# nfmoore/databricks-kubernetes-mlops-poc

Hardware: AMD Instinct MI355X
Metric: requests/sec (whole node), credit-default /score, bs=1024 (higher is better)
Workload: dtype fp32; 1 GPU; model=RandomForest 500xdepth16 + IForest100 + TabularDrift, global_batch=1024, request_rows=1024, with_drift=True, train_rows=20000, parallelism=dp1, device=cuda

## Files before the change

csrc/creditcore_kernels.hip:

```cpp

#include <torch/extension.h>

#include <c10/hip/HIPGuard.h>
#include <c10/hip/HIPStream.h>
#include <hip/hip_runtime.h>

#define BLOCK 256
#define N_CAT 9
#define N_NUM 14
#define MAX_DRIFT_ROWS 16384
static constexpr size_t KS_LDS_BYTES_MAX = 160 * 1024 - 1024;

#define HIP_CHECK(expr)                                              \
  do {                                                               \
    hipError_t _e = (expr);                                          \
    TORCH_CHECK(_e == hipSuccess, "HIP error: ", hipGetErrorString(_e)); \
  } while (0)


template <bool DIRECT>
__global__ __launch_bounds__(BLOCK) void forest_kernel(
    const short* __restrict__ codes,
    const float* __restrict__ nums,
    const float* __restrict__ medians,
// ... 88 lines not shown
    const int ta = t;
    const int tb = t + gridDim.y;
    const int basea = tree_off[ta];
    int4 na = nodes[basea];
    bool la = true;
    int baseb = 0;
    int4 nb;
    bool lb = tb < n_trees;
    if (lb) { baseb = tree_off[tb]; nb = nodes[baseb]; }
    while (la || lb) {
      if (la) {
        if (na.x >= 0) {
          const float v = value_of(na.x);
          na = nodes[basea + ((v <= __int_as_float(na.y)) ? na.z : na.w)];
        } else {
          local += (double)__int_as_float(na.y);
          la = false;
        }
      }
      if (lb) {
        if (nb.x >= 0) {
          const float v = value_of(nb.x);
          nb = nodes[baseb + ((v <= __int_as_float(nb.y)) ? nb.z : nb.w)];
        } else {
          local += (double)__int_as_float(nb.y);
          lb = false;
        }
      }
    }
  }
  atomicAdd(&acc[row], local);
}

template <bool DIRECT>
__device__ __forceinline__ double forest_walk_ilp2(
    const short* __restrict__ s_codes,
    const float* __restrict__ s_nums,
    int tid,
    const int4* __restrict__ nodes,
    const int* __restrict__ tree_off,
    int n_trees,
    const int* __restrict__ feat_col,
    const int* __restrict__ feat_code,
    int chunk,
    int n_chunks)
{
  auto value_of = [&](int f) -> float {
    if (DIRECT) return s_nums[f * BLOCK + tid];
    const int col = feat_col[f];
    const int code = feat_code[f];
    return (code >= 0) ? ((s_codes[col * BLOCK + tid] == (short)code) ? 1.0f : 0.0f)
                       : s_nums[col * BLOCK + tid];
  };
  double local = 0.0;
  for (int t = chunk; t < n_trees; t += 2 * n_chunks) {
    const int ta = t;
    const int tb = t + n_chunks;
    const int basea = tree_off[ta];
    int4 na = nodes[basea];
    bool la = true;
    int baseb = 0;
    int4 nb;
    bool lb = tb < n_trees;
    if (lb) { baseb = tree_off[tb]; nb = nodes[baseb]; }
    while (la || lb) {
      if (la) {
        if (na.x >= 0) {
          const float v = value_of(na.x);
          na = nodes[basea + ((v <= __int_as_float(na.y)) ? na.z : na.w)];
        } else {
          local += (double)__int_as_float(na.y);
          la = false;
        }
      }
      if (lb) {
        if (nb.x >= 0) {
          const float v = value_of(nb.x);
          nb = nodes[baseb + ((v <= __int_as_float(nb.y)) ? nb.z : nb.w)];
        } else {
          local += (double)__int_as_float(nb.y);
          lb = false;
        }
      }
    }
  }
  return local;
}

__global__ __launch_bounds__(BLOCK) void forest_kernel_dual(
    const short* __restrict__ codes,
    const float* __restrict__ nums,
    const float* __restrict__ medians,
    const int4* __restrict__ cls_nodes,
    const int* __restrict__ cls_off,
    int t_cls,
    const int* __restrict__ feat_col,
    const int* __restrict__ feat_code,
    const int4* __restrict__ if_nodes,
    const int* __restrict__ if_off,
    int t_if,
    int chunks_cls,
    int n_rows,
    double* __restrict__ acc_cls,
    double* __restrict__ acc_if)
{
  __shared__ short s_codes[N_CAT * BLOCK];
  __shared__ float s_nums[N_NUM * BLOCK];
  const int tid = threadIdx.x;
  const int row = blockIdx.x * BLOCK + tid;
  const bool is_cls = (int)blockIdx.y < chunks_cls;
  if (row < n_rows) {
    if (is_cls) {
#pragma unroll
      for (int c = 0; c < N_CAT; ++c) s_codes[c * BLOCK + tid] = codes[row * N_CAT + c];
    }
#pragma unroll
    for (int c = 0; c < N_NUM; ++c) {
      const float v = nums[row * N_NUM + c];
      s_nums[c * BLOCK + tid] = isnan(v) ? medians[c] : v;
    }
  }
  if (row >= n_rows) return;
  if (is_cls) {
    const double local = forest_walk_ilp2<false>(
        s_codes, s_nums, tid, cls_nodes, cls_off, t_cls, feat_col, feat_code,
        blockIdx.y, chunks_cls);
    atomicAdd(&acc_cls[row], local);
  } else {
    const double local = forest_walk_ilp2<true>(
        s_codes, s_nums, tid, if_nodes, if_off, t_if, nullptr, nullptr,
        blockIdx.y - chunks_cls, gridDim.y - chunks_cls);
    atomicAdd(&acc_if[row], local);
  }
}

#define CONTRIB_BLOCK 128
#define N_SRC (N_CAT + N_NUM)

__global__ __launch_bounds__(CONTRIB_BLOCK) void forest_contrib_kernel(
    const short* __restrict__ codes,
    const float* __restrict__ nums,
    const float* __restrict__ medians,
    const int4* __restrict__ nodes,
    const float* __restrict__ node_value,
    const int* __restrict__ tree_off,
    int n_trees,
    const int* __restrict__ feat_col,
    const int* __restrict__ feat_code,
    int n_rows,
    double scale,
    double* __restrict__ contrib)
{
  __shared__ double s_acc[N_SRC * CONTRIB_BLOCK];
  __shared__ short s_codes[N_CAT * CONTRIB_BLOCK];
  __shared__ float s_nums[N_NUM * CONTRIB_BLOCK];

  const int tid = threadIdx.x;
  const int row = blockIdx.x * CONTRIB_BLOCK + tid;
  if (row >= n_rows) return;

#pragma unroll
  for (int c = 0; c < N_CAT; ++c)
// ... 2225 lines not shown
  TORCH_CHECK(B <= MAX_DRIFT_ROWS, "K-S batch too large: ", B);
  TORCH_CHECK((int)rs_off.size(0) == F + 1, "rs_off size mismatch");
  TORCH_CHECK(block == 256 || block == 512, "block must be 256 or 512");
  auto ks_d = torch::empty({F},
      torch::TensorOptions().dtype(torch::kFloat32).device(nums.device()));
  hipStream_t stream = c10::hip::getCurrentHIPStream();
  int m_pow2 = (int)block / 64;
  while (m_pow2 < B) m_pow2 <<= 1;
  size_t smem = (size_t)m_pow2 * sizeof(float);
  auto rs_off64 = rs_off.to(torch::kInt64);
  if (ref_lds) {
    int64_t maxr = 0;
    auto ro = rs_off64.cpu();
    auto* rp = ro.data_ptr<int64_t>();
    for (int j = 0; j < F; ++j) maxr = std::max<int64_t>(maxr, rp[j + 1] - rp[j]);
    smem += (size_t)maxr * sizeof(float);
    TORCH_CHECK(smem <= KS_LDS_BYTES_MAX, "ref too large for LDS");
  }
  if (block == 512)
    hipLaunchKernelGGL((ks_kernel_t<512>), dim3(F), dim3(512), smem, stream,
        nums.data_ptr<float>(), medians.data_ptr<float>(), F, B, m_pow2,
        (int)ref_lds, ref_sorted.data_ptr<float>(),
        rs_off64.data_ptr<int64_t>(), ks_d.data_ptr<float>());
  else
    hipLaunchKernelGGL((ks_kernel_t<256>), dim3(F), dim3(256), smem, stream,
        nums.data_ptr<float>(), medians.data_ptr<float>(), F, B, m_pow2,
        (int)ref_lds, ref_sorted.data_ptr<float>(),
        rs_off64.data_ptr<int64_t>(), ks_d.data_ptr<float>());
  HIP_CHECK(hipGetLastError());
  return ks_d;
}


inline bool spin_sync_enabled() {
  static const bool on = (std::getenv("CREDITCORE_BLOCK_SYNC") == nullptr);
  return on;
}

inline void sync_stream(hipStream_t s) {
  if (spin_sync_enabled()) {
    hipError_t e;
    while ((e = hipStreamQuery(s)) == hipErrorNotReady) {}
    if (e != hipSuccess) HIP_CHECK(e);
  } else {
    HIP_CHECK(hipStreamSynchronize(s));
  }
}

inline void sync_event(hipEvent_t ev) {
  static const bool spin = (std::getenv("CREDITCORE_SPIN_EVENT") != nullptr);
  if (spin) {
    hipError_t e;
    while ((e = hipEventQuery(ev)) == hipErrorNotReady) {}
    if (e != hipSuccess) HIP_CHECK(e);
  } else {
    HIP_CHECK(hipEventSynchronize(ev));
  }
}

struct ScoreSession {
  torch::Tensor cls_nodes, cls_off, feat_col, feat_code, medians;
  torch::Tensor if_nodes, if_off, ref_sorted, rs_off, cat_off;
  torch::Tensor d_codes, d_nums, acc, outs, d_drift, d_ks_scratch;
  size_t drift_bytes = 0, drift_ksd_off = 0;
  torch::Tensor pin_codes, pin_nums, pin_outs, pin_drift;
  torch::Tensor pin_hist, pin_ksd;
  double if_denom{}, if_offset{}, if_threshold{};
  int cls_kind{};
  double cls_bias{};
  int64_t total_bins{}, t_cls{}, t_if{}, capacity{};
  int device_index{};
  hipStream_t stream{};
  hipStream_t stream2{};
  hipEvent_t ev_fork{}, ev_join{};
  hipEvent_t ev_done[2]{};

  int16_t* p_codes(int s) { return pin_codes.data_ptr<int16_t>() + (size_t)s * capacity * N_CAT; }
  float* p_nums(int s) { return pin_nums.data_ptr<float>() + (size_t)s * capacity * N_NUM; }
  double* p_outs(int s) { return pin_outs.data_ptr<double>() + (size_t)s * 3 * capacity; }
  uint8_t* p_drift(int s) { return pin_drift.data_ptr<uint8_t>() + (size_t)s * drift_bytes; }
  int32_t* p_hist(int s) { return reinterpret_cast<int32_t*>(p_drift(s)); }
  float* p_ksd(int s) { return reinterpret_cast<float*>(p_drift(s) + drift_ksd_off); }
  int32_t* d_hist() { return reinterpret_cast<int32_t*>(d_drift.data_ptr<uint8_t>()); }
  float* d_ksd() { return reinterpret_cast<float*>(d_drift.data_ptr<uint8_t>() + drift_ksd_off); }

  ScoreSession(py::dict model, int64_t cap, int dev) : capacity(cap), device_index(dev) {
    c10::hip::HIPGuard guard((c10::DeviceIndex)dev);
    auto devopt = torch::TensorOptions().device(torch::kCUDA, dev);
    auto up_i32 = [&](const char* k) {
      return py::cast<torch::Tensor>(model[k]).to(devopt.dtype(torch::kInt32)).contiguous();
    };
    auto up_f32 = [&](const char* k) {
      return py::cast<torch::Tensor>(model[k]).to(devopt.dtype(torch::kFloat32)).contiguous();
    };
    cls_nodes = up_i32("cls_nodes");
// ... 18 lines not shown

    d_codes = torch::empty({capacity, N_CAT}, devopt.dtype(torch::kInt16));
    d_nums = torch::empty({capacity, N_NUM}, devopt.dtype(torch::kFloat32));
    acc = torch::zeros({2, capacity}, devopt.dtype(torch::kFloat64));
    outs = torch::empty({3, capacity}, devopt.dtype(torch::kFloat64));
    drift_ksd_off = (size_t)total_bins * sizeof(int32_t);
    drift_bytes = drift_ksd_off + (size_t)N_NUM * sizeof(float);
    d_drift = torch::empty({(int64_t)drift_bytes}, devopt.dtype(torch::kUInt8));
    d_ks_scratch = torch::empty({(int64_t)N_NUM * KS_MB_MAX_G},
                                devopt.dtype(torch::kFloat32));

    auto pinned = torch::TensorOptions().pinned_memory(true);
    pin_codes = torch::empty({2, capacity, N_CAT}, pinned.dtype(torch::kInt16));
    pin_nums = torch::empty({2, capacity, N_NUM}, pinned.dtype(torch::kFloat32));
    pin_outs = torch::empty({2, 3, capacity}, pinned.dtype(torch::kFloat64));
    pin_drift = torch::empty({2, (int64_t)drift_bytes}, pinned.dtype(torch::kUInt8));
    pin_hist = pin_drift.slice(1, 0, (int64_t)drift_ksd_off).view(torch::kInt32);
    pin_ksd = pin_drift.slice(1, (int64_t)drift_ksd_off, (int64_t)drift_bytes)
                  .view(torch::kFloat32);

    auto rs = py::cast<torch::Tensor>(model["ref_sorted_offsets"]);
    auto rs_acc = rs.accessor<int32_t, 1>();
    for (int j = 0; j + 1 < rs.size(0); ++j)
      max_ref_len = std::max(max_ref_len, (int64_t)(rs_acc[j + 1] - rs_acc[j]));

    (void)hipFuncSetAttribute(reinterpret_cast<const void*>(&ks_kernel_t<256>),
        hipFuncAttributeMaxDynamicSharedMemorySize, (int)KS_LDS_BYTES);
    (void)hipFuncSetAttribute(reinterpret_cast<const void*>(&ks_kernel_t<512>),
        hipFuncAttributeMaxDynamicSharedMemorySize, (int)KS_LDS_BYTES);
    (void)hipFuncSetAttribute(
        reinterpret_cast<const void*>(&ks_count_mb_kernel_t<512>),
        hipFuncAttributeMaxDynamicSharedMemorySize, (int)KS_LDS_BYTES);

    HIP_CHECK(hipStreamCreateWithFlags(&stream, hipStreamNonBlocking));
    HIP_CHECK(hipStreamCreateWithFlags(&stream2, hipStreamNonBlocking));
    HIP_CHECK(hipEventCreateWithFlags(&ev_fork, hipEventDisableTiming));
    HIP_CHECK(hipEventCreateWithFlags(&ev_join, hipEventDisableTiming));
    HIP_CHECK(hipEventCreateWithFlags(&ev_done[0], hipEventDisableTiming));
    HIP_CHECK(hipEventCreateWithFlags(&ev_done[1], hipEventDisableTiming));
    HIP_CHECK(hipDeviceSynchronize());
  }

  ~ScoreSession() {
    if (stream) {
      (void)hipStreamSynchronize(stream);
      for (auto& kv : graphs) (void)hipGraphExecDestroy(kv.second);
      (void)hipStreamDestroy(stream);
      (void)hipStreamDestroy(stream2);
      (void)hipEventDestroy(ev_fork);
      (void)hipEventDestroy(ev_join);
      (void)hipEventDestroy(ev_done[0]);
      (void)hipEventDestroy(ev_done[1]);
    }
  }

  void record(int b, bool with_drift, int slot) {
    HIP_CHECK(hipMemcpyAsync(d_codes.data_ptr(), p_codes(slot),
        (size_t)b * N_CAT * sizeof(short), hipMemcpyHostToDevice, stream));
    HIP_CHECK(hipMemcpyAsync(d_nums.data_ptr(), p_nums(slot),
        (size_t)b * N_NUM * sizeof(float), hipMemcpyHostToDevice, stream));
    const bool fork_drift = with_drift && b > 64;
    hipStream_t sdrift = fork_drift ? stream2 : stream;
    if (fork_drift) {
      HIP_CHECK(hipEventRecord(ev_fork, stream));
      HIP_CHECK(hipStreamWaitEvent(stream2, ev_fork, 0));
    }
    double* acc_cls = acc.data_ptr<double>();
    double* acc_if = acc_cls + b;

    const int row_blocks = ceil_div(b, BLOCK);
    auto chunks = [&](int64_t t) {
      return std::max(1, std::min(ceil_div(2048, row_blocks), (int)((t + 1) / 2)));
    };
    const int c_cls = chunks(t_cls);
    const int c_if = chunks(t_if);
    hipLaunchKernelGGL(forest_kernel_dual, dim3(row_blocks, c_cls + c_if),
        dim3(BLOCK), 0, stream,
        d_codes.data_ptr<short>(), d_nums.data_ptr<float>(), medians.data_ptr<float>(),
        reinterpret_cast<const int4*>(cls_nodes.data_ptr<int>()),
        cls_off.data_ptr<int>(), (int)t_cls,
        feat_col.data_ptr<int>(), feat_code.data_ptr<int>(),
        reinterpret_cast<const int4*>(if_nodes.data_ptr<int>()),
        if_off.data_ptr<int>(), (int)t_if, c_cls, b, acc_cls, acc_if);

    double* proba = outs.data_ptr<double>();
    hipLaunchKernelGGL(finalize_kernel, dim3(row_blocks), dim3(BLOCK), 0, stream,
        acc_cls, acc_if, b, cls_kind, 1.0 / (double)t_cls, cls_bias,
        if_denom, if_offset, if_threshold,
        proba, proba + b, proba + 2 * b);

    if (with_drift) {
      const int hist_blocks = (b <= 2048) ? 1 : std::min(row_blocks, 1024);
      if (hist_blocks > 1)
        HIP_CHECK(hipMemsetAsync(d_hist(), 0, (size_t)total_bins * sizeof(int), sdrift));
      hipLaunchKernelGGL(cat_hist_kernel, dim3(hist_blocks), dim3(BLOCK),
          (size_t)total_bins * sizeof(int), sdrift,
          d_codes.data_ptr<short>(), b, cat_off.data_ptr<int>(), (int)total_bins,
          d_hist());
      if (b <= KS_COUNT_MAX_ROWS) {
        const size_t smem = (size_t)std::max(b, 512 / 64) * sizeof(float);
        hipLaunchKernelGGL((ks_count_kernel_t<512>), dim3(N_NUM), dim3(512),
            smem, sdrift,
            d_nums.data_ptr<float>(), medians.data_ptr<float>(), N_NUM, b,
            ref_sorted.data_ptr<float>(), rs_off.data_ptr<int64_t>(), d_ksd());
      } else if (std::getenv("CREDITCORE_KS_BITONIC") != nullptr) {
        int m_pow2 = 512 / 64;
        while (m_pow2 < b) m_pow2 <<= 1;
        hipLaunchKernelGGL((ks_kernel_t<512>), dim3(N_NUM), dim3(512),
            (size_t)m_pow2 * sizeof(float), sdrift,
            d_nums.data_ptr<float>(), medians.data_ptr<float>(), N_NUM, b,
            m_pow2, 0, ref_sorted.data_ptr<float>(),
            rs_off.data_ptr<int64_t>(), d_ksd());
      } else {
        const int g = ks_mb_blocks(b);
        const size_t smem = (size_t)std::max(b, 512 / 64) * sizeof(float);
        hipLaunchKernelGGL((ks_count_mb_kernel_t<512>), dim3(N_NUM, g),
// ... 657 lines not shown
    } else if (en < 300.0 && d > 0.0 && d < 1.0 && (en * d) * d >= 2.2) {
      p = std::min(1.0, 2.0 * smirnov_sf((int)en, d));
    } else if (en < 500.0 && en * d * std::sqrt(std::max(d, 0.0)) <= 1.4) {
      p = mtw_sf((int)en, d);
    } else {
      p = pelz_good_sf(d, en);
    }
    pv[ncat + j] = p;
  }
}

py::array_t<double> drift_pvals_host(
    py::array_t<int32_t> batch_hist, py::array_t<float> ks_d,
    py::array_t<int32_t> ref_cat_counts, py::array_t<int32_t> cat_offsets,
    int64_t n_ref, int64_t n_batch) {
  const int ncat = (int)cat_offsets.size() - 1;
  const int nnum = (int)ks_d.size();
  py::array_t<double> out({(ssize_t)(ncat + nnum)});
  drift_pvals_raw(batch_hist.data(), ks_d.data(), nnum, ref_cat_counts.data(),
                  cat_offsets.data(), ncat, n_ref, n_batch, out.mutable_data());
  return out;
}

py::tuple encode_json(py::bytes body, py::list vocabs, py::list cat_names,
                      py::list num_names, py::str missing_cat,
                      py::array_t<int16_t> default_codes,
                      py::array_t<float> default_nums) {
  JsonEncoderState st(vocabs, cat_names, num_names, missing_cat,
                      default_codes, default_nums);
  return encode_json_impl(st, body);
}


static inline void append_double(std::string& out, double v) {
  char buf[32];
  auto [p, ec] = std::to_chars(buf, buf + sizeof(buf), v);
  (void)ec;
  bool has_dot = false;
  for (char* c = buf; c < p; ++c)
    if (*c == '.' || *c == 'e' || *c == 'E' || *c == 'n' || *c == 'i') { has_dot = true; break; }
  out.append(buf, p);
  if (!has_dot) out += ".0";
}

py::bytes build_response_json(py::object pin_outs, int64_t b,
                              py::array_t<double> pvals, py::list feature_names) {
  auto outs = py::cast<torch::Tensor>(pin_outs);
  const double* base = outs.data_ptr<double>();
  const double* proba = base;
  const double* outlier = base + 2 * b;
  const int nf = (int)py::len(feature_names);
  const double* pv = pvals.data();

  std::vector<std::string> names(nf);
  for (int j = 0; j < nf; ++j) names[j] = py::cast<std::string>(feature_names[j]);

  std::string out;
  {
    py::gil_scoped_release nogil;
    out.reserve((size_t)b * 24 + 2048);
    out += "{\"predictions\": [";
    for (int64_t i = 0; i < b; ++i) {
      if (i) out += ", ";
      append_double(out, proba[i]);
    }
    out += "], \"outliers\": [";
    for (int64_t i = 0; i < b; ++i) {
      if (i) out += ", ";
      out += (outlier[i] != 0.0) ? "1.0" : "0.0";
    }
    out += "], \"feature_drift_batch\": {";
    for (int j = 0; j < nf; ++j) {
      if (j) out += ", ";
      out += '\"';
      out += names[j];
      out += "\": ";
      append_double(out, (double)(1.0f - (float)pv[j]));
    }
    out += "}}";
  }
  return py::bytes(out);
}

py::bytes build_response_json_arrays(py::array_t<double> predictions,
                                     py::array_t<double> outliers,
                                     py::array_t<double> pvals,
                                     py::list feature_names) {
  const double* proba = predictions.data();
  const double* outl = outliers.data();
  const double* pv = pvals.data();
  const int64_t b = (int64_t)predictions.size();
  TORCH_CHECK((int64_t)outliers.size() == b, "outliers size mismatch");
  const int nf = (int)py::len(feature_names);
  TORCH_CHECK((int)pvals.size() == nf, "pvals size mismatch");
  std::vector<std::string> names(nf);
  for (int j = 0; j < nf; ++j) names[j] = py::cast<std::string>(feature_names[j]);

  std::string out;
  {
    py::gil_scoped_release nogil;
    out.reserve((size_t)b * 24 + 2048);
    out += "{\"predictions\": [";
    for (int64_t i = 0; i < b; ++i) {
      if (i) out += ", ";
      append_double(out, proba[i]);
    }
    out += "], \"outliers\": [";
    for (int64_t i = 0; i < b; ++i) {
      if (i) out += ", ";
      out += (outl[i] != 0.0) ? "1.0" : "0.0";
    }
    out += "], \"feature_drift_batch\": {";
    for (int j = 0; j < nf; ++j) {
      if (j) out += ", ";
      out += '\"';
      out += names[j];
      out += "\": ";
      append_double(out, (double)(1.0f - (float)pv[j]));
    }
    out += "}}";
  }
  return py::bytes(out);
}


py::tuple score_json_full(ScoreSession& s, py::bytes body,
                          const JsonEncoderState& st,
                          py::array_t<int32_t> ref_cat_counts,
                          py::array_t<int32_t> cat_offsets, int64_t n_ref,
                          py::list feature_names, int64_t drift_cap) {
  char* data;
  ssize_t blen;
  if (PyBytes_AsStringAndSize(body.ptr(), &data, &blen) != 0)
    throw py::value_error("body must be bytes");
  const int nf = (int)py::len(feature_names);
  TORCH_CHECK(nf == N_CAT + N_NUM, "feature name count mismatch");
  std::vector<std::string> names(nf);
  for (int j = 0; j < nf; ++j) names[j] = py::cast<std::string>(feature_names[j]);

  std::vector<int16_t> codes;
  std::vector<float> nums;
  size_t b;
  {
    py::gil_scoped_release nogil;
    try {
      b = parse_records_nogil(st, data, blen, codes, nums);
    } catch (const jsonenc::Error& e) {
      py::gil_scoped_acquire gil;
      throw py::value_error(e.msg);
    }
  }
  if (b == 0) throw py::value_error("empty request batch");
  TORCH_CHECK((int64_t)b <= s.capacity, "batch exceeds session capacity: ", b);

  std::memcpy(s.p_codes(0), codes.data(), b * N_CAT * sizeof(int16_t));
  std::memcpy(s.p_nums(0), nums.data(), b * N_NUM * sizeof(float));
  const int64_t cap = (drift_cap > 0) ? std::min<int64_t>(drift_cap, MAX_DRIFT_ROWS)
                                      : MAX_DRIFT_ROWS;
  int64_t nb = (int64_t)b;
  if ((int64_t)b <= cap) {
    s.score((int64_t)b, true, true, 0);
  } else {
    s.score(cap, true, true, 0);
    s.score((int64_t)b, false, true, 0);
    nb = cap;
  }

  double pv[N_CAT + N_NUM];
  drift_pvals_raw(s.p_hist(0), s.p_ksd(0), N_NUM,
                  ref_cat_counts.data(), cat_offsets.data(),
                  (int)cat_offsets.size() - 1, n_ref, nb, pv);

  std::string out;
  {
    py::gil_scoped_release nogil;
    const double* proba = s.p_outs(0);
    const double* outlier = proba + 2 * b;
    out.reserve(b * 24 + 2048);
    out += "{\"predictions\": [";
    for (size_t i = 0; i < b; ++i) {
      if (i) out += ", ";
      append_double(out, proba[i]);
    }
    out += "], \"outliers\": [";
    for (size_t i = 0; i < b; ++i) {
      if (i) out += ", ";
      out += (outlier[i] != 0.0) ? "1.0" : "0.0";
    }
    out += "], \"feature_drift_batch\": {";
    for (int j = 0; j < nf; ++j) {
      if (j) out += ", ";
      out += '\"';
      out += names[j];
      out += "\": ";
      append_double(out, (double)(1.0f - (float)pv[j]));
    }
    out += "}}";
  }
  return py::make_tuple(py::bytes(out), (int64_t)b);
}

void submit_arrays(ScoreSession& s, py::array_t<int16_t> codes,
                   py::array_t<float> nums, int64_t slot, bool with_drift,
                   bool sync) {
  TORCH_CHECK(codes.ndim() == 2 && codes.shape(1) == N_CAT, "codes must be [B, N_CAT]");
  TORCH_CHECK(nums.ndim() == 2 && nums.shape(1) == N_NUM, "nums must be [B, N_NUM]");
  const int64_t b = codes.shape(0);
  TORCH_CHECK(nums.shape(0) == b, "codes/nums row mismatch");
  TORCH_CHECK(b >= 1 && b <= s.capacity, "batch out of range: ", b);
  auto c = codes.unchecked<2>();
  auto n = nums.unchecked<2>();
  const int sl = (int)(slot & 1);
  {
    py::gil_scoped_release nogil;
    int16_t* pc = s.p_codes(sl);
    float* pn = s.p_nums(sl);
    if (codes.strides(0) == (ssize_t)(N_CAT * sizeof(int16_t)) &&
        codes.strides(1) == (ssize_t)sizeof(int16_t)) {
      std::memcpy(pc, c.data(0, 0), (size_t)b * N_CAT * sizeof(int16_t));
    } else {
      for (int64_t i = 0; i < b; ++i)
        for (int j = 0; j < N_CAT; ++j) pc[i * N_CAT + j] = c(i, j);
    }
    if (nums.strides(0) == (ssize_t)(N_NUM * sizeof(float)) &&
        nums.strides(1) == (ssize_t)sizeof(float)) {
      std::memcpy(pn, n.data(0, 0), (size_t)b * N_NUM * sizeof(float));
    } else {
      for (int64_t i = 0; i < b; ++i)
        for (int j = 0; j < N_NUM; ++j) pn[i * N_NUM + j] = n(i, j);
    }
  }
  s.score(b, with_drift, sync, sl);
}

py::bytes response_epilogue(ScoreSession& s, int64_t slot64, int64_t b64,
                            py::array_t<int32_t> ref_cat_counts,
                            py::array_t<int32_t> cat_offsets, int64_t n_ref,
                            py::list feature_names) {
  const int slot = (int)slot64 & 1;
  const int64_t b = b64;
  TORCH_CHECK(b >= 1 && b <= s.capacity, "batch out of range: ", b);
  const int nf = (int)py::len(feature_names);
  std::vector<std::string> names(nf);
  for (int j = 0; j < nf; ++j) names[j] = py::cast<std::string>(feature_names[j]);
  const int64_t nb = std::min<int64_t>(b, MAX_DRIFT_ROWS);

  double pv[N_CAT + N_NUM];
  std::string out;
  {
    py::gil_scoped_release nogil;
    sync_event(s.ev_done[slot]);
    drift_pvals_raw(s.p_hist(slot), s.p_ksd(slot), N_NUM,
                    ref_cat_counts.data(), cat_offsets.data(),
                    (int)cat_offsets.size() - 1, n_ref, nb, pv);
    const double* proba = s.p_outs(slot);
    const double* outlier = proba + 2 * b;
    out.reserve((size_t)b * 24 + 2048);
    out += "{\"predictions\": [";
    for (int64_t i = 0; i < b; ++i) {
      if (i) out += ", ";
      append_double(out, proba[i]);
    }
    out += "], \"outliers\": [";
    for (int64_t i = 0; i < b; ++i) {
      if (i) out += ", ";
      out += (outlier[i] != 0.0) ? "1.0" : "0.0";
    }
    out += "], \"feature_drift_batch\": {";
    for (int j = 0; j < nf; ++j) {
      if (j) out += ", ";
      out += '\"';
      out += names[j];
      out += "\": ";
      append_double(out, (double)(1.0f - (float)pv[j]));
    }
    out += "}}";
  }
  return py::bytes(out);
}

PYBIND11_MODULE(TORCH_EXTENSION_NAME, m) {
  m.def("score_forest_pipeline", &score_forest_pipeline,
        "Forest classifier + isolation forest scoring (gfx950)");
  m.def("forest_contrib", &forest_contrib,
        "Per-row prediction-path feature attributions f64[B,23] (gfx950)",
        py::arg("codes"), py::arg("nums"), py::arg("cls_nodes"),
        py::arg("cls_node_value"), py::arg("cls_off"), py::arg("feat_col"),
        py::arg("feat_code"), py::arg("medians"), py::arg("cls_kind"),
        py::arg("block_target") = 512);
  m.def("forest_shap", &forest_shap,
        "Per-row exact TreeSHAP feature attributions f64[B,23] (gfx950)",
        py::arg("codes"), py::arg("nums"), py::arg("leaf_value"),
        py::arg("leaf_off"), py::arg("splits"), py::arg("medians"),
        py::arg("cls_kind"), py::arg("n_trees"),
        py::arg("block_target") = 2048);
  m.def("forest_shap_interactions", &forest_shap_interactions,
        "Per-row exact SHAP interaction values f64[B,23,23], diagonal left "
        "at zero (gfx950)",
        py::arg("codes"), py::arg("nums"), py::arg("leaf_value"),
        py::arg("leaf_off"), py::arg("splits"), py::arg("medians"),
        py::arg("cls_kind"), py::arg("n_trees"),
        py::arg("block_target") = 2048);
  m.attr("SHAP_INTER_ROWS_PER_BLOCK") = py::int_(SHAPI_ROWS);
  m.def("forest_ishap", &forest_ishap,
        "Per-row interventional Shapley values f64[B,23] against a "
        "background sample (gfx950)",
        py::arg("codes"), py::arg("nums"), py::arg("bg_codes"),
        py::arg("bg_nums"), py::arg("leaf_value"), py::arg("leaf_off"),
        py::arg("splits"), py::arg("medians"), py::arg("cls_kind"),
        py::arg("n_trees"), py::arg("block_target") = 2048);
  m.attr("ISHAP_MAX_BACKGROUND") = py::int_(ISHAP_MAX_BACKGROUND);
  m.def("hgbt_hist", &hgbt_hist,
        "HistGBT level histogram i64[n_nodes,3,total_bins] of int32 "
        "fixed-point gradients (gfx950)",
// ... 50 lines not shown
  m.def("ks_stats_sorted", &ks_stats_sorted,
        "Exact K-S D per column for pre-sorted batch columns (gfx950)");
  m.def("forest_ilp_bench", &forest_ilp_bench,
        "A/B: forest traversal, 1 vs 2 trees per thread");
  m.def("ks_stats", &ks_stats,
        "Exact two-sample K-S D per column, any column count (gfx950)",
        py::arg("nums"), py::arg("medians"), py::arg("ref_sorted"),
        py::arg("rs_off"), py::arg("block") = 256, py::arg("ref_lds") = 0);
  m.def("build_response_json", &build_response_json,
        "Serialize the /score response to JSON bytes (C, shortest doubles)");
  m.def("build_response_json_arrays", &build_response_json_arrays,
        "Serialize a /score response from plain arrays (merged-flush slices)");
  m.def("drift_pvals_host", &drift_pvals_host,
        "Drift p-values from kernel statistics (chi2 + Pelz-Good K-S), host C");
  py::class_<ScoreSession>(m, "ScoreSession")
      .def(py::init<py::dict, int64_t, int>(), py::arg("model"),
           py::arg("capacity"), py::arg("device_index"))
      .def("score", &ScoreSession::score, py::arg("b"),
           py::arg("with_drift") = true, py::arg("sync") = true,
           py::arg("slot") = 0)
      .def("wait_slot", &ScoreSession::wait_slot)
      .def("submit_arrays", &submit_arrays, py::arg("codes"), py::arg("nums"),
           py::arg("slot") = 0, py::arg("with_drift") = true,
           py::arg("sync") = false)
      .def("response_epilogue", &response_epilogue, py::arg("slot"),
           py::arg("b"), py::arg("ref_cat_counts"), py::arg("cat_offsets"),
           py::arg("n_ref"), py::arg("feature_names"))
      .def("synchronize", &ScoreSession::synchronize)
      .def("score_json_full", &score_json_full, py::arg("body"),
           py::arg("encoder"), py::arg("ref_cat_counts"),
           py::arg("cat_offsets"), py::arg("n_ref"), py::arg("feature_names"),
           py::arg("drift_cap") = -1)
      .def_readonly("capacity", &ScoreSession::capacity)
      .def_property_readonly("pin_codes", [](ScoreSession& s) { return s.pin_codes; })
      .def_property_readonly("pin_nums", [](ScoreSession& s) { return s.pin_nums; })
      .def_property_readonly("pin_outs", [](ScoreSession& s) { return s.pin_outs; })
      .def_property_readonly("pin_hist", [](ScoreSession& s) { return s.pin_hist; })
      .def_property_readonly("pin_ksd", [](ScoreSession& s) { return s.pin_ksd; });
}
```

Baseline: 8817 requests/s.

## Resolve forest split features into node table and write JSON directly into bytes

At session setup the classifier and isolation forest node tables are rebuilt on the host. Each split node's feature index is replaced by a packed word holding the column, the category code and a one-hot flag, so the traversal kernel no longer does two dependent global loads (feat_col/feat_code) per split. An optional blocked layout packs subtrees into 128-byte slots, selectable by env var; the default is the resolved layout without blocking. The response JSON writer also now writes directly into a preallocated Python bytes buffer instead of growing a std::string and copying it, which removes one copy and the reallocations. This adds setup-time host work and extra device memory for the duplicated tables.

```diff
diff --git a/csrc/creditcore_kernels.hip b/csrc/creditcore_kernels.hip
--- a/csrc/creditcore_kernels.hip
+++ b/csrc/creditcore_kernels.hip
@@ -144,7 +144,12 @@
   atomicAdd(&acc[row], local);
 }
 
-template <bool DIRECT>
+#define RN_CODE_MASK 0xFFFF
+#define RN_COL_SHIFT 16
+#define RN_COL_MASK 0xFF
+#define RN_ONEHOT_BIT (1 << 24)
+
+template <bool DIRECT, bool RESOLVED>
 __device__ __forceinline__ double forest_walk_ilp2(
     const short* __restrict__ s_codes,
     const float* __restrict__ s_nums,
@@ -159,6 +164,12 @@
 {
   auto value_of = [&](int f) -> float {
     if (DIRECT) return s_nums[f * BLOCK + tid];
+    if (RESOLVED) {
+      const int col = (f >> RN_COL_SHIFT) & RN_COL_MASK;
+      return (f & RN_ONEHOT_BIT)
+                 ? ((s_codes[col * BLOCK + tid] == (short)(f & RN_CODE_MASK)) ? 1.0f : 0.0f)
+                 : s_nums[col * BLOCK + tid];
+    }
     const int col = feat_col[f];
     const int code = feat_code[f];
     return (code >= 0) ? ((s_codes[col * BLOCK + tid] == (short)code) ? 1.0f : 0.0f)
@@ -199,6 +210,7 @@
   return local;
 }
 
+template <bool RESOLVED>
 __global__ __launch_bounds__(BLOCK) void forest_kernel_dual(
     const short* __restrict__ codes,
     const float* __restrict__ nums,
@@ -234,12 +246,12 @@
   }
   if (row >= n_rows) return;
   if (is_cls) {
-    const double local = forest_walk_ilp2<false>(
+    const double local = forest_walk_ilp2<false, RESOLVED>(
         s_codes, s_nums, tid, cls_nodes, cls_off, t_cls, feat_col, feat_code,
         blockIdx.y, chunks_cls);
     atomicAdd(&acc_cls[row], local);
   } else {
-    const double local = forest_walk_ilp2<true>(
+    const double local = forest_walk_ilp2<true, RESOLVED>(
         s_codes, s_nums, tid, if_nodes, if_off, t_if, nullptr, nullptr,
         blockIdx.y - chunks_cls, gridDim.y - chunks_cls);
     atomicAdd(&acc_if[row], local);
@@ -2531,6 +2543,141 @@
 }
 
 
+
+#include <deque>
+#include <stdexcept>
+
+#define RELAYOUT_BLOCK_SLOTS 8
+#define RELAYOUT_BLOCK_NODES 7
+static constexpr double RELAYOUT_MAX_GROWTH = 2.0;
+
+struct RelayoutStats {
+  int64_t n_nodes = 0;
+  int64_t n_slots = 0;
+  int64_t n_blocks = 0;
+  double fill = 1.0;
+  bool resolved = false;
+  bool blocked = false;
+  bool guard_tripped = false;
+};
+
+static const char* const FOREST_TABLES_DEFAULT = "resolved";
+
+static inline int32_t relayout_resolve_feat(int32_t col, int32_t code) {
+  return (code >= 0 ? RN_ONEHOT_BIT : 0) | ((col & RN_COL_MASK) << RN_COL_SHIFT) |
+         (code & RN_CODE_MASK);
+}
+
+static RelayoutStats relayout_forest_host(
+    const int32_t* nodes, int64_t n_nodes, const int32_t* off, int64_t n_trees,
+    const int32_t* feat_col, const int32_t* feat_code, int64_t n_feat,
+    bool direct, bool resolve, bool block,
+    std::vector<int32_t>& out_nodes, std::vector<int32_t>& out_off,
+    double max_growth = RELAYOUT_MAX_GROWTH)
+{
+  auto bad = [](const char* what) { throw std::invalid_argument(std::string("relayout_forest: ") + what); };
+  if (n_trees < 1 || off[0] != 0 || off[n_trees] != n_nodes) bad("tree offsets do not cover the node table");
+  resolve = resolve && !direct;
+  if (resolve) {
+    for (int64_t f = 0; f < n_feat; ++f) {
+      if (feat_code[f] < -32768 || feat_code[f] > 32767) bad("feat_code outside int16");
+      const int lim = feat_code[f] >= 0 ? N_CAT : N_NUM;
+      if (feat_col[f] < 0 || feat_col[f] >= lim) bad("feat_col out of range");
+    }
+  }
+  const int64_t n_feat_eff = direct ? N_NUM : n_feat;
+  for (int64_t t = 0; t < n_trees; ++t) {
+    const int64_t size = (int64_t)off[t + 1] - off[t];
+    if (size < 1) bad("empty tree");
+    for (int64_t k = off[t]; k < off[t + 1]; ++k) {
+      const int32_t* nd = nodes + 4 * k;
+      if (nd[0] < 0) continue;
+      if (nd[0] >= n_feat_eff) bad("split feature out of range");
+      if (nd[2] < 0 || nd[2] >= size || nd[3] < 0 || nd[3] >= size) bad("child outside its tree");
+    }
+  }
+
+  RelayoutStats st;
+  st.n_nodes = n_nodes;
+  st.resolved = resolve;
+  const int32_t zero_leaf[4] = {-1, 0 , 0, 0};
+  auto emit = [&](const int32_t* nd, int32_t left, int32_t right) {
+    int32_t feat = nd[0];
+    if (feat >= 0 && resolve) feat = relayout_resolve_feat(feat_col[feat], feat_code[feat]);
+    out_nodes.insert(out_nodes.end(), {feat, nd[1], feat >= 0 ? left : nd[2], feat >= 0 ? right : nd[3]});
+  };
+
+  std::vector<int32_t> slot_of;
+  std::vector<int32_t> new_idx(n_nodes, -1);
+  std::vector<int64_t> tree_slot0(n_trees + 1, 0);
+  bool use_blocks = block;
+  if (block) {
+    slot_of.reserve((size_t)n_nodes * 2);
+    std::deque<int32_t> roots, q;
+    for (int64_t t = 0; t < n_trees && use_blocks; ++t) {
+      const int32_t* tn = nodes + 4 * (int64_t)off[t];
+      int32_t* tnew = new_idx.data() + off[t];
+      const int64_t slot0 = (int64_t)slot_of.size();
+      tree_slot0[t] = slot0;
+      roots.assign(1, 0);
+      while (!roots.empty()) {
+        const int64_t block0 = (int64_t)slot_of.size() - slot0;
+        q.assign(1, roots.front());
+        roots.pop_front();
+        int count = 0;
+        while (!q.empty() && count < RELAYOUT_BLOCK_NODES) {
+          const int32_t n = q.front();
+          q.pop_front();
+          if (tnew[n] >= 0) bad("node reachable along two paths");
+          tnew[n] = (int32_t)(block0 + count);
+          slot_of.push_back(n);
+          ++count;
+          if (tn[4 * n] >= 0) { q.push_back(tn[4 * n + 2]); q.push_back(tn[4 * n + 3]); }
+        }
+        roots.insert(roots.end(), q.begin(), q.end());
+        slot_of.resize((size_t)(slot0 + block0 + RELAYOUT_BLOCK_SLOTS), -1);
+        ++st.n_blocks;
+        if ((double)slot_of.size() > max_growth * (double)n_nodes) { use_blocks = false; break; }
+      }
+    }
+    tree_slot0[n_trees] = (int64_t)slot_of.size();
+    if (use_blocks && (int64_t)slot_of.size() > INT32_MAX) use_blocks = false;
+    st.guard_tripped = !use_blocks;
+  }
+
+  out_nodes.clear();
+  out_off.assign(n_trees + 1, 0);
+  if (use_blocks) {
+    out_nodes.reserve(slot_of.size() * 4);
+    int64_t live = 0;
+    for (int64_t t = 0; t < n_trees; ++t) {
+      const int32_t* tn = nodes + 4 * (int64_t)off[t];
+      const int32_t* tnew = new_idx.data() + off[t];
+      out_off[t] = (int32_t)tree_slot0[t];
+      for (int64_t s = tree_slot0[t]; s < tree_slot0[t + 1]; ++s) {
+        const int32_t n = slot_of[s];
+        if (n < 0) { emit(zero_leaf, 0, 0); continue; }
+        const int32_t* nd = tn + 4 * n;
+        ++live;
+        if (nd[0] >= 0) emit(nd, tnew[nd[2]], tnew[nd[3]]);
+        else emit(nd, 0, 0);
+      }
+    }
+    out_off[n_trees] = (int32_t)tree_slot0[n_trees];
+    st.blocked = true;
+    st.n_slots = (int64_t)slot_of.size();
+    st.fill = st.n_slots ? (double)live / (double)st.n_slots : 1.0;
+  } else {
+    out_nodes.reserve((size_t)n_nodes * 4);
+    for (int64_t k = 0; k < n_nodes; ++k) emit(nodes + 4 * k, nodes[4 * k + 2], nodes[4 * k + 3]);
+    for (int64_t t = 0; t <= n_trees; ++t) out_off[t] = off[t];
+    st.n_blocks = 0;
+    st.n_slots = n_nodes;
+    st.fill = 1.0;
+  }
+  return st;
+}
+
 inline bool spin_sync_enabled() {
   static const bool on = (std::getenv("CREDITCORE_BLOCK_SYNC") == nullptr);
   return on;
@@ -2560,6 +2707,9 @@
 struct ScoreSession {
   torch::Tensor cls_nodes, cls_off, feat_col, feat_code, medians;
   torch::Tensor if_nodes, if_off, ref_sorted, rs_off, cat_off;
+  torch::Tensor cls_nodes2, cls_off2, if_nodes2, if_off2;
+  bool tables_packed = false;
+  RelayoutStats cls_layout, if_layout;
   torch::Tensor d_codes, d_nums, acc, outs, d_drift, d_ks_scratch;
   size_t drift_bytes = 0, drift_ksd_off = 0;
   torch::Tensor pin_codes, pin_nums, pin_outs, pin_drift;
@@ -2644,6 +2794,42 @@
         reinterpret_cast<const void*>(&ks_count_mb_kernel_t<512>),
         hipFuncAttributeMaxDynamicSharedMemorySize, (int)KS_LDS_BYTES);
 
+    {
+      const char* env = std::getenv("CREDITCORE_FOREST_TABLES");
+      const std::string form = (env && *env) ? env : FOREST_TABLES_DEFAULT;
+      TORCH_CHECK(form == "packed" || form == "resolved" || form == "blocked",
+                  "CREDITCORE_FOREST_TABLES must be packed, resolved or blocked, got: ",
+                  form);
+      tables_packed = form == "packed";
+      auto host_i32 = [&](const char* k) {
+        return py::cast<torch::Tensor>(model[k]).to(torch::kCPU, torch::kInt32).contiguous();
+      };
+      auto build = [&](const char* kn, const char* ko, bool direct, bool block,
+                       torch::Tensor& nodes2, torch::Tensor& off2) {
+        auto n = host_i32(kn), o = host_i32(ko);
+        auto fcol = host_i32("feat_col"), fcode = host_i32("feat_code");
+        TORCH_CHECK(fcol.numel() == fcode.numel(), "feat_col/feat_code size mismatch");
+        std::vector<int32_t> on, oo;
+        RelayoutStats st = relayout_forest_host(
+            n.data_ptr<int32_t>(), n.numel() / 4, o.data_ptr<int32_t>(), o.numel() - 1,
+            fcol.data_ptr<int32_t>(), fcode.data_ptr<int32_t>(), fcol.numel(),
+            direct, true, block, on, oo);
+        nodes2 = torch::from_blob(on.data(), {(int64_t)on.size() / 4, 4}, torch::kInt32)
+                     .to(devopt.dtype(torch::kInt32)).contiguous();
+        off2 = torch::from_blob(oo.data(), {(int64_t)oo.size()}, torch::kInt32)
+                   .to(devopt.dtype(torch::kInt32)).contiguous();
+        TORCH_CHECK(reinterpret_cast<uintptr_t>(nodes2.data_ptr()) % 128 == 0,
+                    "traversal table is not 128-byte aligned");
+        return st;
+      };
+      if (!tables_packed) {
+        cls_layout = build("cls_nodes", "cls_tree_offsets", false, form == "blocked",
+                           cls_nodes2, cls_off2);
+        if_layout = build("if_nodes", "if_tree_offsets", true, form == "blocked",
+                          if_nodes2, if_off2);
+      }
+    }
+
     HIP_CHECK(hipStreamCreateWithFlags(&stream, hipStreamNonBlocking));
     HIP_CHECK(hipStreamCreateWithFlags(&stream2, hipStreamNonBlocking));
     HIP_CHECK(hipEventCreateWithFlags(&ev_fork, hipEventDisableTiming));
@@ -2686,14 +2872,25 @@
     };
     const int c_cls = chunks(t_cls);
     const int c_if = chunks(t_if);
-    hipLaunchKernelGGL(forest_kernel_dual, dim3(row_blocks, c_cls + c_if),
-        dim3(BLOCK), 0, stream,
-        d_codes.data_ptr<short>(), d_nums.data_ptr<float>(), medians.data_ptr<float>(),
-        reinterpret_cast<const int4*>(cls_nodes.data_ptr<int>()),
-        cls_off.data_ptr<int>(), (int)t_cls,
-        feat_col.data_ptr<int>(), feat_code.data_ptr<int>(),
-        reinterpret_cast<const int4*>(if_nodes.data_ptr<int>()),
-        if_off.data_ptr<int>(), (int)t_if, c_cls, b, acc_cls, acc_if);
+    if (tables_packed) {
+      hipLaunchKernelGGL(forest_kernel_dual<false>, dim3(row_blocks, c_cls + c_if),
+          dim3(BLOCK), 0, stream,
+          d_codes.data_ptr<short>(), d_nums.data_ptr<float>(), medians.data_ptr<float>(),
+          reinterpret_cast<const int4*>(cls_nodes.data_ptr<int>()),
+          cls_off.data_ptr<int>(), (int)t_cls,
+          feat_col.data_ptr<int>(), feat_code.data_ptr<int>(),
+          reinterpret_cast<const int4*>(if_nodes.data_ptr<int>()),
+          if_off.data_ptr<int>(), (int)t_if, c_cls, b, acc_cls, acc_if);
+    } else {
+      hipLaunchKernelGGL(forest_kernel_dual<true>, dim3(row_blocks, c_cls + c_if),
+          dim3(BLOCK), 0, stream,
+          d_codes.data_ptr<short>(), d_nums.data_ptr<float>(), medians.data_ptr<float>(),
+          reinterpret_cast<const int4*>(cls_nodes2.data_ptr<int>()),
+          cls_off2.data_ptr<int>(), (int)t_cls,
+          (const int*)nullptr, (const int*)nullptr,
+          reinterpret_cast<const int4*>(if_nodes2.data_ptr<int>()),
+          if_off2.data_ptr<int>(), (int)t_if, c_cls, b, acc_cls, acc_if);
+    }
 
     double* proba = outs.data_ptr<double>();
     hipLaunchKernelGGL(finalize_kernel, dim3(row_blocks), dim3(BLOCK), 0, stream,
@@ -3417,54 +3614,88 @@
 }
 
 
-static inline void append_double(std::string& out, double v) {
-  char buf[32];
-  auto [p, ec] = std::to_chars(buf, buf + sizeof(buf), v);
-  (void)ec;
-  bool has_dot = false;
-  for (char* c = buf; c < p; ++c)
-    if (*c == '.' || *c == 'e' || *c == 'E' || *c == 'n' || *c == 'i') { has_dot = true; break; }
-  out.append(buf, p);
-  if (!has_dot) out += ".0";
-}
+static constexpr size_t RESPONSE_DOUBLE_MAX = 26;
+
+static inline char* put_double(char* p, double v) {
+  char* e = std::to_chars(p, p + 32, v).ptr;
+  for (const char* c = p; c < e; ++c)
+    if (*c == '.' || *c == 'e' || *c == 'E' || *c == 'n' || *c == 'i') return e;
+  *e++ = '.';
+  *e++ = '0';
+  return e;
+}
+
+template <size_t N>
+static inline char* put_lit(char* p, const char (&s)[N]) {
+  std::memcpy(p, s, N - 1);
+  return p + (N - 1);
+}
+
+struct ResponseWriter {
+  std::vector<std::string> names;
+  py::bytes holder;
+  char* buf = nullptr;
+  int64_t b = 0;
+
+  ResponseWriter(py::list feature_names, int64_t b_) : b(b_) {
+    const size_t nf = py::len(feature_names);
+    names.resize(nf);
+    size_t bound = 128 + (size_t)b * (RESPONSE_DOUBLE_MAX + 2 + 5);
+    for (size_t j = 0; j < nf; ++j) {
+      names[j] = py::cast<std::string>(feature_names[j]);
+      bound += names[j].size() + 6 + RESPONSE_DOUBLE_MAX;
+    }
+    PyObject* o = PyBytes_FromStringAndSize(nullptr, (Py_ssize_t)bound);
+    if (!o) throw py::error_already_set();
+    holder = py::reinterpret_steal<py::bytes>(o);
+    buf = PyBytes_AS_STRING(o);
+  }
+
+  size_t write(const double* proba, const double* outlier, const double* pv) const {
+    char* p = put_lit(buf, "{\"predictions\": [");
+    for (int64_t i = 0; i < b; ++i) {
+      if (i) p = put_lit(p, ", ");
+      p = put_double(p, proba[i]);
+    }
+    p = put_lit(p, "], \"outliers\": [");
+    for (int64_t i = 0; i < b; ++i) {
+      if (i) p = put_lit(p, ", ");
+      p = (outlier[i] != 0.0) ? put_lit(p, "1.0") : put_lit(p, "0.0");
+    }
+    p = put_lit(p, "], \"feature_drift_batch\": {");
+    for (size_t j = 0; j < names.size(); ++j) {
+      if (j) p = put_lit(p, ", ");
+      *p++ = '\"';
+      std::memcpy(p, names[j].data(), names[j].size());
+      p += names[j].size();
+      p = put_lit(p, "\": ");
+      p = put_double(p, (double)(1.0f - (float)pv[j]));
+    }
+    p = put_lit(p, "}}");
+    return (size_t)(p - buf);
+  }
+
+  py::bytes finish(size_t len) {
+    PyObject* o = holder.release().ptr();
+    if (_PyBytes_Resize(&o, (Py_ssize_t)len) != 0) throw py::error_already_set();
+    return py::reinterpret_steal<py::bytes>(o);
+  }
+};
 
 py::bytes build_response_json(py::object pin_outs, int64_t b,
                               py::array_t<double> pvals, py::list feature_names) {
   auto outs = py::cast<torch::Tensor>(pin_outs);
+  TORCH_CHECK(b >= 0 && 3 * b <= outs.numel(), "batch out of range: ", b);
   const double* base = outs.data_ptr<double>();
-  const double* proba = base;
-  const double* outlier = base + 2 * b;
-  const int nf = (int)py::len(feature_names);
+  ResponseWriter w(feature_names, b);
+  TORCH_CHECK((size_t)pvals.size() == w.names.size(), "pvals size mismatch");
   const double* pv = pvals.data();
-
-  std::vector<std::string> names(nf);
-  for (int j = 0; j < nf; ++j) names[j] = py::cast<std::string>(feature_names[j]);
-
-  std::string out;
+  size_t len;
   {
     py::gil_scoped_release nogil;
-    out.reserve((size_t)b * 24 + 2048);
-    out += "{\"predictions\": [";
-    for (int64_t i = 0; i < b; ++i) {
-      if (i) out += ", ";
-      append_double(out, proba[i]);
-    }
-    out += "], \"outliers\": [";
-    for (int64_t i = 0; i < b; ++i) {
-      if (i) out += ", ";
-      out += (outlier[i] != 0.0) ? "1.0" : "0.0";
-    }
-    out += "], \"feature_drift_batch\": {";
-    for (int j = 0; j < nf; ++j) {
-      if (j) out += ", ";
-      out += '\"';
-      out += names[j];
-      out += "\": ";
-      append_double(out, (double)(1.0f - (float)pv[j]));
-    }
-    out += "}}";
-  }
-  return py::bytes(out);
+    len = w.write(base, base + 2 * b, pv);
+  }
+  return w.finish(len);
 }
 
 py::bytes build_response_json_arrays(py::array_t<double> predictions,
@@ -3476,36 +3707,14 @@
   const double* pv = pvals.data();
   const int64_t b = (int64_t)predictions.size();
   TORCH_CHECK((int64_t)outliers.size() == b, "outliers size mismatch");
-  const int nf = (int)py::len(feature_names);
-  TORCH_CHECK((int)pvals.size() == nf, "pvals size mismatch");
-  std::vector<std::string> names(nf);
-  for (int j = 0; j < nf; ++j) names[j] = py::cast<std::string>(feature_names[j]);
-
-  std::string out;
+  ResponseWriter w(feature_names, b);
+  TORCH_CHECK((size_t)pvals.size() == w.names.size(), "pvals size mismatch");
+  size_t len;
   {
     py::gil_scoped_release nogil;
-    out.reserve((size_t)b * 24 + 2048);
-    out += "{\"predictions\": [";
-    for (int64_t i = 0; i < b; ++i) {
-      if (i) out += ", ";
-      append_double(out, proba[i]);
-    }
-    out += "], \"outliers\": [";
-    for (int64_t i = 0; i < b; ++i) {
-      if (i) out += ", ";
-      out += (outl[i] != 0.0) ? "1.0" : "0.0";
-    }
-    out += "], \"feature_drift_batch\": {";
-    for (int j = 0; j < nf; ++j) {
-      if (j) out += ", ";
-      out += '\"';
-      out += names[j];
-      out += "\": ";
-      append_double(out, (double)(1.0f - (float)pv[j]));
-    }
-    out += "}}";
-  }
-  return py::bytes(out);
+    len = w.write(proba, outl, pv);
+  }
+  return w.finish(len);
 }
 
 
@@ -3520,8 +3729,6 @@
     throw py::value_error("body must be bytes");
   const int nf = (int)py::len(feature_names);
   TORCH_CHECK(nf == N_CAT + N_NUM, "feature name count mismatch");
-  std::vector<std::string> names(nf);
-  for (int j = 0; j < nf; ++j) names[j] = py::cast<std::string>(feature_names[j]);
 
   std::vector<int16_t> codes;
   std::vector<float> nums;
@@ -3556,33 +3763,14 @@
                   ref_cat_counts.data(), cat_offsets.data(),
                   (int)cat_offsets.size() - 1, n_ref, nb, pv);
 
-  std::string out;
+  ResponseWriter w(feature_names, (int64_t)b);
+  size_t len;
   {
     py::gil_scoped_release nogil;
     const double* proba = s.p_outs(0);
-    const double* outlier = proba + 2 * b;
-    out.reserve(b * 24 + 2048);
-    out += "{\"predictions\": [";
-    for (size_t i = 0; i < b; ++i) {
-      if (i) out += ", ";
-      append_double(out, proba[i]);
-    }
-    out += "], \"outliers\": [";
-    for (size_t i = 0; i < b; ++i) {
-      if (i) out += ", ";
-      out += (outlier[i] != 0.0) ? "1.0" : "0.0";
-    }
-    out += "], \"feature_drift_batch\": {";
-    for (int j = 0; j < nf; ++j) {
-      if (j) out += ", ";
-      out += '\"';
-      out += names[j];
-      out += "\": ";
-      append_double(out, (double)(1.0f - (float)pv[j]));
-    }
-    out += "}}";
-  }
-  return py::make_tuple(py::bytes(out), (int64_t)b);
+    len = w.write(proba, proba + 2 * b, pv);
+  }
+  return py::make_tuple(w.finish(len), (int64_t)b);
 }
 
 void submit_arrays(ScoreSession& s, py::array_t<int16_t> codes,
@@ -3625,13 +3813,12 @@
   const int slot = (int)slot64 & 1;
   const int64_t b = b64;
   TORCH_CHECK(b >= 1 && b <= s.capacity, "batch out of range: ", b);
-  const int nf = (int)py::len(feature_names);
-  std::vector<std::string> names(nf);
-  for (int j = 0; j < nf; ++j) names[j] = py::cast<std::string>(feature_names[j]);
+  ResponseWriter w(feature_names, b);
+  TORCH_CHECK(w.names.size() <= (size_t)(N_CAT + N_NUM), "feature name count mismatch");
   const int64_t nb = std::min<int64_t>(b, MAX_DRIFT_ROWS);
 
   double pv[N_CAT + N_NUM];
-  std::string out;
+  size_t len;
   {
     py::gil_scoped_release nogil;
     sync_event(s.ev_done[slot]);
@@ -3639,32 +3826,99 @@
                     ref_cat_counts.data(), cat_offsets.data(),
                     (int)cat_offsets.size() - 1, n_ref, nb, pv);
     const double* proba = s.p_outs(slot);
-    const double* outlier = proba + 2 * b;
-    out.reserve((size_t)b * 24 + 2048);
-    out += "{\"predictions\": [";
-    for (int64_t i = 0; i < b; ++i) {
-      if (i) out += ", ";
-      append_double(out, proba[i]);
-    }
-    out += "], \"outliers\": [";
-    for (int64_t i = 0; i < b; ++i) {
-      if (i) out += ", ";
-      out += (outlier[i] != 0.0) ? "1.0" : "0.0";
-    }
-    out += "], \"feature_drift_batch\": {";
-    for (int j = 0; j < nf; ++j) {
-      if (j) out += ", ";
-      out += '\"';
-      out += names[j];
-      out += "\": ";
-      append_double(out, (double)(1.0f - (float)pv[j]));
-    }
-    out += "}}";
-  }
-  return py::bytes(out);
+    len = w.write(proba, proba + 2 * b, pv);
+  }
+  return w.finish(len);
+}
+
+static py::dict relayout_stats_dict(const RelayoutStats& st) {
+  py::dict d;
+  d["n_nodes"] = st.n_nodes;
+  d["n_slots"] = st.n_slots;
+  d["n_blocks"] = st.n_blocks;
+  d["bytes"] = st.n_slots * (int64_t)sizeof(int4);
+  d["fill_ratio"] = st.fill;
+  d["resolved"] = st.resolved;
+  d["blocked"] = st.blocked;
+  d["guard_tripped"] = st.guard_tripped;
+  return d;
+}
+
+using i32_array = py::array_t<int32_t, py::array::c_style | py::array::forcecast>;
+
+py::tuple relayout_forest(i32_array nodes, i32_array tree_offsets,
+                          i32_array feat_col, i32_array feat_code, bool direct,
+                          bool resolve, bool block, double max_growth) {
+  if (nodes.ndim() != 2 || nodes.shape(1) != 4) throw py::value_error("nodes must be [n, 4]");
+  if (tree_offsets.ndim() != 1 || tree_offsets.size() < 2)
+    throw py::value_error("tree_offsets must be [T + 1], T >= 1");
+  if (feat_col.size() != feat_code.size()) throw py::value_error("feat_col/feat_code size mismatch");
+  std::vector<int32_t> on, oo;
+  RelayoutStats st;
+  try {
+    st = relayout_forest_host(nodes.data(), nodes.shape(0), tree_offsets.data(),
+                              tree_offsets.size() - 1, feat_col.data(), feat_code.data(),
+                              feat_col.size(), direct, resolve, block, on, oo, max_growth);
+  } catch (const std::invalid_argument& e) {
+    throw py::value_error(e.what());
+  }
+  py::array_t<int32_t> n2({(py::ssize_t)(on.size() / 4), (py::ssize_t)4});
+  py::array_t<int32_t> o2((py::ssize_t)oo.size());
+  std::memcpy(n2.mutable_data(), on.data(), on.size() * sizeof(int32_t));
+  std::memcpy(o2.mutable_data(), oo.data(), oo.size() * sizeof(int32_t));
+  return py::make_tuple(n2, o2, relayout_stats_dict(st));
+}
+
+torch::Tensor forest_dual_bench(
+    torch::Tensor codes, torch::Tensor nums, torch::Tensor medians,
+    torch::Tensor cls_nodes, torch::Tensor cls_off,
+    torch::Tensor feat_col, torch::Tensor feat_code,
+    torch::Tensor if_nodes, torch::Tensor if_off, bool resolved)
+{
+  check_inputs(codes, nums);
+  for (const auto& t : {cls_nodes, cls_off, feat_col, feat_code, if_nodes, if_off})
+    TORCH_CHECK(t.is_cuda() && t.is_contiguous() && t.dtype() == torch::kInt32,
+                "forest tables must be contiguous int32 CUDA tensors");
+  TORCH_CHECK(medians.is_cuda() && medians.dtype() == torch::kFloat32 &&
+              medians.numel() == N_NUM, "medians must be f32[N_NUM] on the GPU");
+  const int B = (int)codes.size(0);
+  const int t_cls = (int)cls_off.size(0) - 1, t_if = (int)if_off.size(0) - 1;
+  TORCH_CHECK(t_cls >= 1 && t_if >= 1, "empty forest");
+  auto acc = torch::zeros({2, B},
+      torch::TensorOptions().dtype(torch::kFloat64).device(codes.device()));
+  hipStream_t stream = c10::hip::getCurrentHIPStream();
+  const int row_blocks = ceil_div(B, BLOCK);
+  auto chunks = [&](int t) {
+    return std::max(1, std::min(ceil_div(2048, row_blocks), (t + 1) / 2));
+  };
+  const int c_cls = chunks(t_cls), c_if = chunks(t_if);
+  auto launch = [&](auto kernel) {
+    hipLaunchKernelGGL(kernel, dim3(row_blocks, c_cls + c_if), dim3(BLOCK), 0, stream,
+        codes.data_ptr<short>(), nums.data_ptr<float>(), medians.data_ptr<float>(),
+        reinterpret_cast<const int4*>(cls_nodes.data_ptr<int>()), cls_off.data_ptr<int>(), t_cls,
+        feat_col.data_ptr<int>(), feat_code.data_ptr<int>(),
+        reinterpret_cast<const int4*>(if_nodes.data_ptr<int>()), if_off.data_ptr<int>(), t_if,
+        c_cls, B, acc.data_ptr<double>(), acc.data_ptr<double>() + B);
+  };
+  if (resolved) launch(forest_kernel_dual<true>);
+  else launch(forest_kernel_dual<false>);
+  HIP_CHECK(hipGetLastError());
+  return acc;
 }
 
 PYBIND11_MODULE(TORCH_EXTENSION_NAME, m) {
+  m.def("relayout_forest", &relayout_forest,
+        "Session traversal table of a packed forest: resolved features and/or "
+        "128-byte line blocking (host)",
+        py::arg("nodes"), py::arg("tree_offsets"), py::arg("feat_col"),
+        py::arg("feat_code"), py::arg("direct"), py::arg("resolve") = true,
+        py::arg("block") = true, py::arg("max_growth") = RELAYOUT_MAX_GROWTH);
+  m.def("forest_dual_bench", &forest_dual_bench,
+        "A/B: one forest_kernel_dual launch over packed or resolved tables, "
+        "raw accumulators f64[2,B]",
+        py::arg("codes"), py::arg("nums"), py::arg("medians"), py::arg("cls_nodes"),
+        py::arg("cls_off"), py::arg("feat_col"), py::arg("feat_code"),
+        py::arg("if_nodes"), py::arg("if_off"), py::arg("resolved"));
   m.def("score_forest_pipeline", &score_forest_pipeline,
         "Forest classifier + isolation forest scoring (gfx950)");
   m.def("forest_contrib", &forest_contrib,
@@ -3781,6 +4035,15 @@
            py::arg("cat_offsets"), py::arg("n_ref"), py::arg("feature_names"),
            py::arg("drift_cap") = -1)
       .def_readonly("capacity", &ScoreSession::capacity)
+      .def_property_readonly("forest_tables", [](ScoreSession& s) {
+        py::dict d;
+        d["packed"] = s.tables_packed;
+        if (!s.tables_packed) {
+          d["cls"] = relayout_stats_dict(s.cls_layout);
+          d["if"] = relayout_stats_dict(s.if_layout);
+        }
+        return d;
+      })
       .def_property_readonly("pin_codes", [](ScoreSession& s) { return s.pin_codes; })
       .def_property_readonly("pin_nums", [](ScoreSession& s) { return s.pin_nums; })
       .def_property_readonly("pin_outs", [](ScoreSession& s) { return s.pin_outs; })
```

Result: slower. 7525 requests/s (-14.6%).
